# tum-vision/dvo_slam

Measured on NVIDIA H100. Metric: frame-pair alignments/sec @640x480x5-level, higher is better.
Workload: dtype f32

## Files before the change

dvo_slam_b200/csrc/stages.cuh:

```cuda
#pragma once
#include "common.cuh"
#include "f32x2.cuh"

namespace dvo_b200 {

constexpr unsigned kFullMask = 0xffffffffu;
constexpr int kConsumerWarps = kTileH;
constexpr int kCtaThreads = (kConsumerWarps + 1) * 32;
#ifndef DVO_WIN_COLS
#define DVO_WIN_COLS 152
#endif
#ifndef DVO_WIN_ROWS
#define DVO_WIN_ROWS 24
#endif
#ifndef DVO_STAGES
#define DVO_STAGES 2
#endif
constexpr int kWinCols = DVO_WIN_COLS;
constexpr int kWinRows = DVO_WIN_ROWS;
constexpr int kStages = DVO_STAGES;

__device__ __forceinline__ unsigned smem_u32(const void* p) { return (unsigned)__cvta_generic_to_shared(p); }
__device__ __forceinline__ void mbar_init(unsigned long long* bar, unsigned count) {
  asm volatile("mbarrier.init.shared::cta.b64 [%0], %1;" ::"r"(smem_u32(bar)), "r"(count) : "memory");
// ... 41 lines not shown
#if DVO_TRYWAIT_HINT_NS > 0
  asm volatile(
      "{\n\t.reg .pred p;\n\tmbarrier.try_wait.parity.acquire.cta.shared::cta.b64 p, [%1], %2, %3;\n\tselp.u32 %0, 1, 0, p;\n\t}"
      : "=r"(ok)
      : "r"(bar), "r"(parity), "r"((unsigned)DVO_TRYWAIT_HINT_NS)
      : "memory");
#else
  asm volatile(
      "{\n\t.reg .pred p;\n\tmbarrier.try_wait.parity.acquire.cta.shared::cta.b64 p, [%1], %2;\n\tselp.u32 %0, 1, 0, p;\n\t}"
      : "=r"(ok)
      : "r"(bar), "r"(parity)
      : "memory");
#endif
  return ok != 0;
}
__device__ __forceinline__ void mbar_wait_s(unsigned bar, unsigned parity, int* error_flag) {
  unsigned spins = 0;
  while (!mbar_try_wait_s(bar, parity)) {
    if (((++spins) & 0xfffu) == 0u) {
      if (*reinterpret_cast<volatile int*>(error_flag)) break;
      if (spins > (1u << 24)) { atomicExch(error_flag, 2); break; }
    }
  }
}
__device__ __forceinline__ void mbar_arrive_s(unsigned bar) {
  asm volatile("{\n\t.reg .b64 st;\n\tmbarrier.arrive.release.cta.shared::cta.b64 st, [%0];\n\t}" ::"r"(bar) : "memory");
}
__device__ __forceinline__ int4 lds_i4(unsigned addr) {
  int4 v;
  asm volatile("ld.shared.v4.b32 {%0, %1, %2, %3}, [%4];" : "=r"(v.x), "=r"(v.y), "=r"(v.z), "=r"(v.w) : "r"(addr));
  return v;
}

__device__ __forceinline__ void bulk_g2s(void* dst_smem, const void* src_gmem, unsigned bytes, unsigned long long* bar) {
  asm volatile("cp.async.bulk.shared::cta.global.mbarrier::complete_tx::bytes [%0], [%1], %2, [%3];" ::"r"(smem_u32(dst_smem)),
               "l"(src_gmem), "r"(bytes), "r"(smem_u32(bar))
               : "memory");
}
// ... 10 lines not shown
  return v;
}
__device__ __forceinline__ f2 lds_f2_at(unsigned addr) {
  f2 v;
  asm volatile("ld.shared.v2.f32 {%0, %1}, [%2];" : "=f"(v.x), "=f"(v.y) : "r"(addr));
  return v;
}

__device__ __forceinline__ unsigned pin(unsigned v) { asm volatile("" : "+r"(v)); return v; }
__device__ __forceinline__ int pin(int v) { asm volatile("" : "+r"(v)); return v; }
__device__ __forceinline__ float pin(float v) { asm volatile("" : "+f"(v)); return v; }
template <typename T>
__device__ __forceinline__ const T* pin(const T* p) { asm volatile("" : "+l"(p)); return p; }

struct __align__(16) TileDesc {
  int skip;
  int origin;
  int ulo, ucount;
  int vlo, vcount;
  int exact;
  int cmask;
};
struct __align__(128) StageBuf {
  float2 ref0[kTileH][kTileW];
  float tx[kTileW];
  float2 ref1[kTileH][kTileW];
  float2 win[kWinRows][kWinCols];
};
static_assert(offsetof(StageBuf, tx) == kRecTx * sizeof(float2) && offsetof(StageBuf, ref1) == kRecP1 * sizeof(float2) &&
              offsetof(StageBuf, win) == kRecF2 * sizeof(float2), "StageBuf must mirror the reference tile record");
struct TilePipe {
  StageBuf buf[kStages];
  unsigned long long full[kStages], empty[kStages];
  TileDesc desc[kStages];
};
static_assert(sizeof(TileDesc) == 32 && offsetof(TilePipe, desc) % 16 == 0, "TileDesc is read as two 16-byte words");

#ifdef DVO_PIPE_TIMING
struct PipeTiming {
  unsigned long long wait_full_a = 0, wait_full_b = 0, wait_empty = 0, produce = 0, rounds_a = 0, rounds_b = 0;
  unsigned long long tiles = 0, tiles_inexact = 0, tiles_skipped = 0, tiles_cmask = 0, slow_rounds = 0, rounds = 0;
  bool on = false;
};
#define DVO_CLOCK(tm) ((tm).on ? clock64() : 0)
#define DVO_ADD(tm, field, v) do { if ((tm).on) (tm).field += (v); } while (0)
#else
struct PipeTiming {};
#define DVO_CLOCK(tm) 0ll
#define DVO_ADD(tm, field, v) do { } while (0)
#endif

struct LevelGeom {
  int w, h, n, pitch;
  int nbands, nstrips;
  int strip0, strip_step, nmine;
};

struct StageConsts {
  f2 k0, k1, k2, k3;
  float k8, k9, k10, k11;
  f2 Pa, Pb;
  f2 cgh, cg, fxyh;
  float c_i, ubx, uby;
  int first_iteration;
};

__device__ __forceinline__ void load_stage_consts(const PairState& st, const PairLevel& pl, int w, int h, bool weights_from_prev,
                                                  StageConsts& c) {
  float kt[12], P[4];
#pragma unroll
  for (int i = 0; i < 12; ++i) kt[i] = __ldcg(&st.kt[i]);
#pragma unroll
  for (int i = 0; i < 4; ++i) P[i] = weights_from_prev ? __ldcg(&st.precision_prev[i]) : __ldcg(&st.precision[i]);
  c.k0 = pk(kt[0], kt[4]); c.k1 = pk(kt[1], kt[5]); c.k2 = pk(kt[2], kt[6]); c.k3 = pk(kt[3], kt[7]);
  c.k8 = kt[8]; c.k9 = kt[9]; c.k10 = kt[10]; c.k11 = kt[11];
  c.Pa = pk(P[0], P[1]); c.Pb = pk(P[2], P[3]);
  const float cgx = __fdiv_rn(__fmul_rn(0.5f, pl.cfx), 255.0f), cgy = __fdiv_rn(__fmul_rn(0.5f, pl.cfy), 255.0f);
  c.cg = pk(cgx, cgy);
  c.cgh = pk(0.5f * cgx, 0.5f * cgy);
  c.fxyh = pk(0.5f * pl.cfx, 0.5f * pl.cfy);
  c.c_i = 1.0f / 255.0f;
  c.ubx = pin((float)(w - 2)); c.uby = pin((float)(h - 2));
  c.first_iteration = __ldcg(&st.iteration) == 0;
}

template <bool kStageB, bool kCurMask = false>
__device__ __noinline__ void produce_tiles(TilePipe& tp, const PairLevel& pl, const LevelGeom& g, const StageConsts& c, unsigned tbase,
                                           int ntiles, int* error_flag, PipeTiming& tm) {
  const int lane = threadIdx.x & 31, sub = lane >> 3;
  const float2* cur = kStageB ? pl.c3 : pl.c0;
  int s_issue = g.strip0, b_issue = 0;
  for (int i0 = 0; i0 < ntiles; i0 += 4) {
    const long long tp0 = DVO_CLOCK(tm);
    unsigned wordA, wordD;
    {
      const int ii = min(i0 + sub, ntiles - 1);
      const int sd = ii / g.nbands;
      const int s = g.strip0 + sd * g.strip_step, b = ii - sd * g.nbands;
      const int y0 = s * kTileH, rows = min(kTileH, g.h - y0);
      const int x0 = b * kTileW, bw = min(kTileW, g.w - x0);
      const float2 zr = __ldg(pl.rrange + (size_t)s * g.nbands + b);
      const float txc = __ldg(pl.rtmpl + ((lane & 1) ? x0 + bw - 1 : x0));
      const float tyc = __ldg(pl.rtmpl + g.w + ((lane & 2) ? y0 + rows - 1 : y0));
      const bool has_depth = zr.x <= zr.y;
      const float z = (lane & 4) ? zr.y : zr.x;
      const float px = txc * z, py = tyc * z;
      const f2 XY = fma2(c.k0, bc(px), fma2(c.k1, bc(py), fma2(c.k2, bc(z), c.k3)));
      const float Zt = fmaf(c.k8, px, fmaf(c.k9, py, fmaf(c.k10, z, c.k11)));
      const float iz = 1.0f / Zt;
      float umin = lo(XY) * iz, vmin = hi(XY) * iz, umax = umin, vmax = vmin;
      const bool front_lane = Zt > 1e-6f && umin == umin && vmin == vmin;
#pragma unroll
      for (int off = 1; off < 8; off <<= 1) {
        umin = fminf(umin, __shfl_xor_sync(kFullMask, umin, off)); umax = fmaxf(umax, __shfl_xor_sync(kFullMask, umax, off));
        vmin = fminf(vmin, __shfl_xor_sync(kFullMask, vmin, off)); vmax = fmaxf(vmax, __shfl_xor_sync(kFullMask, vmax, off));
      }
      const bool front = ((__ballot_sync(kFullMask, front_lane) >> (sub * 8)) & 0xffu) == 0xffu;
      umin = fmaxf(umin, -8.f); vmin = fmaxf(vmin, -8.f); umax = fminf(umax, (float)g.w + 8.f); vmax = fminf(vmax, (float)g.h + 8.f);
// ... 24 lines not shown
        if (exact) {
          const int cx0 = bx0 >> 3, cx1 = (min(bx0 + ncols - 1, g.w - 1) >> 3) + 1;
          const int cy0 = max(row_lo, 0) >> 3, cy1 = (min(row_lo + nrows - 1, g.h - 1) >> 3) + 1;
          const int dirty = __ldg(csat + cy1 * sw + cx1) - __ldg(csat + cy0 * sw + cx1) - __ldg(csat + cy1 * sw + cx0) +
                            __ldg(csat + cy0 * sw + cx0);
          if (dirty) { exact = 0; cmask = 1; }
        } else {
          cmask = __ldg(csat + (sat_rows(g.h) - 1) * sw + sw - 1) != 0 ? 1 : 0;
        }
      }
      wordA = (unsigned)skip | ((unsigned)exact << 1) | ((unsigned)ncols << 2) | ((unsigned)nrows << 10) | ((unsigned)cmask << 31);
      wordD = (unsigned)bx0 | ((unsigned)(row_lo + 1) << 16);
    }
    DVO_ADD(tm, produce, DVO_CLOCK(tm) - tp0);
    const int kmax = min(4, ntiles - i0);
    for (int k = 0; k < kmax; ++k) {
      const unsigned t = tbase + (unsigned)(i0 + k);
      const int bufi = t % kStages;
      StageBuf& sb = tp.buf[bufi];
      const unsigned wa = __shfl_sync(kFullMask, wordA, k * 8), wd = __shfl_sync(kFullMask, wordD, k * 8);
      const int s = s_issue, b = b_issue;
      if (++b_issue == g.nbands) { b_issue = 0; s_issue += g.strip_step; }
      const int skip = (int)(wa & 1u), ncols = (int)((wa >> 2) & 0xffu), nrows = (int)((kCurMask ? wa & 0x7fffffffu : wa) >> 10);
      const int win_bx0 = (int)(wd & 0xffffu), win_row_lo = (int)(wd >> 16) - 1;
      TileDesc d;
      d.skip = skip; d.exact = (int)((wa >> 1) & 1u); d.cmask = kCurMask ? (int)(wa >> 31) : 0;
      d.origin = 0; d.ulo = 0; d.ucount = 0; d.vlo = 0; d.vcount = 0;
      if (ncols) {
        d.origin = (win_row_lo * kWinCols + win_bx0) * 8;
        d.ulo = win_bx0 == 0 ? 0 : win_bx0 + 1;
        const int uhi = (win_bx0 + ncols - 1 >= g.w - 1) ? g.w - 2 : win_bx0 + ncols - 3;
        d.ucount = max(uhi - d.ulo + 1, 0);
        d.vlo = win_row_lo + 1;
        d.vcount = max(nrows - 3, 0);
      }
      const unsigned win_row_bytes = (unsigned)ncols * 8u;
      const unsigned rec_bytes = (unsigned)(kStageB ? kRecF2 : kRecP1) * 8u;
      const unsigned total = skip ? 0u : rec_bytes + (unsigned)nrows * win_row_bytes;
      const long long tp1 = DVO_CLOCK(tm);
      mbar_wait(&tp.empty[bufi], ((t / kStages) & 1u) ^ 1u, error_flag);
      DVO_ADD(tm, wait_empty, DVO_CLOCK(tm) - tp1);
      DVO_ADD(tm, tiles, 1); DVO_ADD(tm, tiles_inexact, (!d.skip && !d.exact) ? 1 : 0); DVO_ADD(tm, tiles_skipped, d.skip ? 1 : 0);
      DVO_ADD(tm, tiles_cmask, d.cmask ? 1 : 0);
      if (lane == 0) {
        tp.desc[bufi] = d;
        if (total) mbar_arrive_expect_tx(&tp.full[bufi], total);
        else mbar_arrive(&tp.full[bufi]);
      }
      __syncwarp();
      if (!skip) {
        if (lane < nrows) {
          const int yy = min(max(win_row_lo + lane, 0), g.h - 1);
          bulk_g2s(&sb.win[lane][0], cur + (size_t)yy * g.pitch + win_bx0, win_row_bytes, &tp.full[bufi]);
        }
        if (lane == 31) bulk_g2s(&sb.ref0[0][0], pl.r0 + (size_t)(s * g.nbands + b) * kRecF2, rec_bytes, &tp.full[bufi]);
      }
    }
  }
}

struct PixelProjection {
  f2 f, gq;
  float Zt;
  int u0, v0;
  bool inb;
};

__device__ __forceinline__ PixelProjection project_pixel(float tx, float ty, float z, const StageConsts& c) {
  PixelProjection p;
  const f2 pxy = mul2(pk(tx, ty), bc(z));
  const float px = lo(pxy), py = hi(pxy);
  const f2 XY = fma2(c.k0, bc(px), fma2(c.k1, bc(py), fma2(c.k2, bc(z), c.k3)));
  p.Zt = __fmaf_rn(c.k8, px, __fmaf_rn(c.k9, py, __fmaf_rn(c.k10, z, c.k11)));
// ... 395 lines not shown
    }
    if (kCorrected && !kExact) {
      z0 = (r * 32 + lane == odd_col) ? odd_z : z0;
      z1 = (r * 32 + 32 + lane == odd_col) ? odd_z : z1;
    }
    const PixelProjection p0 = project_pixel(tx0, ty, z0, c);
    const PixelProjection p1 = project_pixel(tx1, ty, z1, c);
    float ei0, ez0, ei1, ez1;
    const bool v0 = residual_pixel<kExact>(p0, wv, ref_intensity<kAffine>(lo(rz0), br), z0, c, ei0, ez0);
    const bool v1 = residual_pixel<kExact>(p1, wv, ref_intensity<kAffine>(lo(rz1), br), z1, c, ei1, ez1);
    const float w0 = student_weight(c, first, ei0, ez0), w1 = student_weight(c, first, ei1, ez1);
    scale_add(ss, lane, lt_mask, v0, w0, ei0, ez0);
    scale_add(ss, lane, lt_mask, v1, w1, ei1, ez1);
  }
}
template <bool kCorrected, bool kAffine = false>
__device__ __forceinline__ void stage_a_run(TilePipe& tp, const PairLevel& pl, const LevelGeom& g, const StageConsts& c,
                                            float* row_exports, unsigned& tile_count, int* error_flag, PipeTiming& tm,
                                            const Brightness& br = {1.f, 0.f}) {
  const int lane = threadIdx.x & 31, q = threadIdx.x >> 5;
  const unsigned lt_mask = (1u << lane) - 1u;
  const int ntiles = g.nmine * g.nbands;
  const unsigned tbase = tile_count;
  tile_count += ntiles;
  if (q == kConsumerWarps) {
    produce_tiles<false>(tp, pl, g, c, tbase, ntiles, error_flag, tm);
    return;
  }
  int i = 0;
  const unsigned tp_s = pin(smem_u32(&tp));
  const unsigned my_ref = pin((unsigned)(offsetof(StageBuf, ref0) + (q * kTileW + lane) * 8));
  const unsigned my_tx = pin((unsigned)(offsetof(StageBuf, tx) + lane * 4));
  const int gw = pin(g.w), gh = pin(g.h), gnb = pin(g.nbands), gpitch = g.pitch;
  OddPoint odd;
  odd.y = -1; odd.x = 0; odd.z = 0.f;
  if (kCorrected) odd = load_odd_point(pl, g);
  for (int sk = 0, s = g.strip0; sk < g.nmine; ++sk, s += g.strip_step) {
    const int y = s * kTileH + q;
    const bool row_ok = y < gh;
    const float ty = __ldg(pl.rtmpl + gw + min(y, gh - 1));
    typename ScaleOf<kCorrected>::type ss;
    scale_state_init(ss);
    for (int b = 0; b < gnb; ++b, ++i) {
      const unsigned t = tbase + i;
      const unsigned bufi = t % kStages;
      const int x0 = b * kTileW, bw = min(kTileW, gw - x0);
      const long long tw0 = DVO_CLOCK(tm);
      mbar_wait_s(tp_s + (unsigned)offsetof(TilePipe, full) + bufi * 8u, (t / kStages) & 1u, error_flag);
      DVO_ADD(tm, wait_full_a, DVO_CLOCK(tm) - tw0);
      const unsigned bufs = tp_s + bufi * (unsigned)sizeof(StageBuf);
      const int4 d0 = lds_i4(tp_s + (unsigned)offsetof(TilePipe, desc) + bufi * 32u);
      if (row_ok && !d0.x) {
        const int4 d1 = lds_i4(tp_s + (unsigned)offsetof(TilePipe, desc) + bufi * 32u + 16u);
        const WinView wv = make_view(bufs, d0, d1, pl.c0, gw, gh, gpitch);
        const unsigned refa = bufs + my_ref, txa = bufs + my_tx;
        const bool odd_tile = kCorrected && y == odd.y && (unsigned)(odd.x - x0) < (unsigned)bw;
        if (wv.exact && bw == kTileW && !odd_tile) {
          if (c.first_iteration) stage_a_rounds<kCorrected, true, true, kAffine>(wv, bw, refa, txa, ty, c, ss, lane, lt_mask, -1, 0.f, br);
          else stage_a_rounds<kCorrected, true, false, kAffine>(wv, bw, refa, txa, ty, c, ss, lane, lt_mask, -1, 0.f, br);
        } else {
          stage_a_rounds<kCorrected, false, false, kAffine>(wv, bw, refa, txa, ty, c, ss, lane, lt_mask, odd_tile ? odd.x - x0 : -1,
                                                            odd.z, br);
        }
      }
      __syncwarp();
      if (lane == 0) mbar_arrive_s(tp_s + (unsigned)offsetof(TilePipe, empty) + bufi * 8u);
    }
    if (row_ok) scale_state_export(ss, lane, row_exports + (size_t)y * kSegExportFloats);
  }
}

struct StageBConsts {
  float P00, P01, P10, P11;
  float l, wd0, wd1;
};

template <int kCols> constexpr int kNormalValuesOf = 1 + kCols * (kCols + 1) / 2 + kCols;
constexpr int kNormalValues = kNormalValuesOf<6>;
constexpr int kNormalValuesAffine = kNormalValuesOf<8>;
template <bool kAffine> constexpr int kColsOf = kAffine ? 8 : 6;

template <int kCols>
__host__ __device__ constexpr int tri(int r, int c) { return r * kCols - r * (r - 1) / 2 + (c - r); }
template <int kCols>
// ... 145 lines not shown
      keep = valid && (rank + __popc(m & lt_mask)) < keep_rank;
      rank += __popc(m);
    }
    if (kDump && r * 32 < xlim) dump_record(dump, pix + r * 32, valid, E, G, H, z);
    const float ei = valid ? lo(E) : 0.f, ez = valid ? hi(E) : 0.f;
    const float wall = student_weight(c, first, ei, ez);
    const float wgt = valid ? wall : 0.f;
    stage_b_pixel(acc, cb, wgt, keep, ei, ez, valid ? G : bc(0.f), valid ? H : bc(0.f), valid ? z : 1.0f, valid ? tx : 0.f, ty,
                  valid ? lo(rz) : 0.f, -c.c_i);
  }
}

template <bool kDump, bool kCorrected, bool kCurMask = false, bool kAffine = false>
__device__ __forceinline__ void stage_b_run(TilePipe& tp, const PairLevel& pl, const LevelGeom& g, const StageConsts& c,
                                            const StageBConsts& cb, const int* row_base, const int* strip_base, long long n_keep,
                                            const RecordDump& dump, float* row_partial, unsigned& tile_count, int* error_flag,
                                            PipeTiming& tm, const Brightness& br = {1.f, 0.f}) {
  constexpr int kCols = kColsOf<kAffine>;
  const int lane = threadIdx.x & 31, q = threadIdx.x >> 5;
  const unsigned lt_mask = (1u << lane) - 1u;
  const int ntiles = g.nmine * g.nbands;
  const unsigned tbase = tile_count;
  tile_count += ntiles;
  if (q == kConsumerWarps) {
    produce_tiles<true, kCurMask>(tp, pl, g, c, tbase, ntiles, error_flag, tm);
    return;
  }
  int i = 0;
  const unsigned tp_s = pin(smem_u32(&tp));
  const unsigned my_ref = (unsigned)(offsetof(StageBuf, ref0) + (q * kTileW + lane) * 8);
  const unsigned my_tx = (unsigned)(offsetof(StageBuf, tx) + lane * 4);
  const int gw = g.w, gh = g.h, gnb = g.nbands, gpitch = g.pitch;
  OddPoint odd;
  odd.y = -1; odd.x = 0; odd.z = 0.f;
  if (kCorrected) odd = load_odd_point(pl, g);
  for (int sk = 0, s = g.strip0; sk < g.nmine; ++sk, s += g.strip_step) {
    const int y = s * kTileH + q;
    const bool row_ok = y < gh;
    const float ty = __ldg(pl.rtmpl + gw + min(y, gh - 1));
    bool cta_has_tail = false;
    int keep_rank = 0;
    int rank = 0;
    if (!kCorrected) {
      const long long sbase = __ldcg(strip_base + s);
      cta_has_tail = (long long)__ldcg(strip_base + s + 1) > n_keep;
      keep_rank = (int)max(min(n_keep - sbase, (long long)0x7fffffff), (long long)-1);
      if (cta_has_tail && row_ok) rank = __ldcg(row_base + y);
    }
    StageBAccN<kCols> acc;
    stage_b_init(acc);
    for (int b = 0; b < gnb; ++b, ++i) {
      const unsigned t = tbase + i;
      const unsigned bufi = t % kStages;
      const int x0 = b * kTileW, bw = min(kTileW, gw - x0);
      const long long tw0 = DVO_CLOCK(tm);
      mbar_wait_s(tp_s + (unsigned)offsetof(TilePipe, full) + bufi * 8u, (t / kStages) & 1u, error_flag);
      DVO_ADD(tm, wait_full_b, DVO_CLOCK(tm) - tw0);
      const unsigned bufs = tp_s + bufi * (unsigned)sizeof(StageBuf);
      const int4 d0 = lds_i4(tp_s + (unsigned)offsetof(TilePipe, desc) + bufi * 32u);
      if (row_ok && !d0.x) {
        const int4 d1 = lds_i4(tp_s + (unsigned)offsetof(TilePipe, desc) + bufi * 32u + 16u);
        const WinView wv = make_view(bufs, d0, d1, pl.c3, gw, gh, gpitch);
        const unsigned refa = bufs + my_ref, txa = bufs + my_tx;
        const size_t pix = (size_t)y * gw + x0 + lane;
        const bool odd_tile = kCorrected && y == odd.y && (unsigned)(odd.x - x0) < (unsigned)bw;
        if (wv.exact && bw == kTileW && !cta_has_tail && !odd_tile) {
          if (c.first_iteration)
            stage_b_rounds<kCorrected, true, true, kDump, false, kAffine>(wv, bw, refa, txa, ty, c, cb, acc, cta_has_tail, rank, keep_rank,
                                                                          dump, pix, lane, lt_mask, -1, 0.f, tm, false, nullptr, br);
          else
            stage_b_rounds<kCorrected, true, false, kDump, false, kAffine>(wv, bw, refa, txa, ty, c, cb, acc, cta_has_tail, rank, keep_rank,
                                                                           dump, pix, lane, lt_mask, -1, 0.f, tm, false, nullptr, br);
        } else {
          stage_b_rounds<kCorrected, false, false, kDump, kCurMask, kAffine>(wv, bw, refa, txa, ty, c, cb, acc, cta_has_tail, rank,
                                                                             keep_rank, dump, pix, lane, lt_mask,
                                                                             odd_tile ? odd.x - x0 : -1, odd.z, tm,
                                                                             kCurMask && d1.w != 0, pl.c0, br);
        }
      } else if (kDump && row_ok) {
        for (int xl = lane; xl < bw; xl += 32) dump_record(dump, (size_t)y * gw + x0 + xl, false, bc(0.f), bc(0.f), bc(0.f), 0.f);
      }
      __syncwarp();
      if (lane == 0) mbar_arrive_s(tp_s + (unsigned)offsetof(TilePipe, empty) + bufi * 8u);
    }
    if (row_ok) flush_row_partial(acc, lane, row_partial + (size_t)y * kNormalValuesOf<kCols>);
  }
}

__device__ __forceinline__ void load_stage_b_consts(const PairState& st, StageBConsts& c) {
  c.P00 = __ldcg(&st.precision[0]); c.P01 = __ldcg(&st.precision[1]); c.P10 = __ldcg(&st.precision[2]); c.P11 = __ldcg(&st.precision[3]);
  c.l = c.P01 / c.P00;
  c.wd0 = c.P00;
  c.wd1 = c.P11 - c.P01 * c.l;
}

}
```

dvo_slam_b200/csrc/tracker.cu:

```cuda
#include "common.cuh"
#include "stages.cuh"
#include "launch_plan.h"

#include <cstdio>
#include <cstring>
#include <limits>
#include <cmath>
#include <cstdlib>
#include <algorithm>
#include <type_traits>

namespace dvo_b200 {

namespace {

constexpr unsigned kFull = 0xffffffffu;
constexpr int kEndWarps = 4;

struct LevelLaunch {
  int w, h, n, pitch;
  int nbands, nstrips;
  int level_index;
  int level_id;
  int max_iterations;
// ... 349 lines not shown
    ls.has_inc = ls.num_iterations >= need;
  } else {
    st.inc = inc;
    st.initial_old = st.initial;
    st.initial = se3_mul(se3_inverse(inc), st.initial);
    st.estimate_old = st.estimate;
    st.estimate = estimate_new;
  }
  phase(5);
}

struct SquadState {
  int pair;
  unsigned arrive;
  unsigned phase;
  int pad_[29];
};

template <bool kAffine, bool kPrior = false>
struct LevelTailOf {
  using EndBase = typename std::conditional<kAffine, PairEndSmemAffine, PairEndSmem>::type;
  SegCombineSmem comb;
  typename std::conditional<kPrior, PairEndSmemPrior<EndBase>, EndBase>::type end;
  int s_flag[2];
};
template <bool kAffine, bool kPrior = false>
constexpr size_t kLevelSmemBytesOf = sizeof(TilePipe) + sizeof(LevelTailOf<kAffine, kPrior>);
constexpr size_t kLevelSmemBytes = kLevelSmemBytesOf<false>;

struct Segment {
  const PairLevel* pls;
  float* row_exports;
  int* row_base;
  double* strip_exports;
  int* strip_base;
  float* row_partial;
  double* strip_partial;
  SquadState* squads;
  int* queue;
  int* ready;
  int* ready_tail;
  int* arrivals;
  int cyclic;
  int pair_begin;
  int npairs_seg;
  unsigned long long* dbg2;
  unsigned long long* dbg;
  int nlev;
  int g, nsquads;
  int strips_per_cta[kMaxLevels];
  LevelLaunch lp[kMaxLevels];
};

struct PersistentArgs {
  PairState* states;
  int* error_flag;
  dvo_b200_iteration_stats* ilog;
  int max_log;
  const double* T_init;
  int skip_begin;
  float* dump;
  int npairs;
  int nseg;
  Segment seg[kMaxSeg];
  const PairLevel* pls0;
// ... 93 lines not shown
    cta_index = lt.s_flag[1];
    __syncthreads();
  }
  const int squad = cta_index / S.g, rank = cta_index - squad * S.g;
  if (squad >= S.nsquads) continue;
  SquadState* sq = S.squads + squad;
  int hmax = 0;
  for (int li = 0; li < S.nlev; ++li) hmax = max(hmax, S.lp[li].h);
  float* row_exports = S.row_exports + (size_t)squad * hmax * kSegExportFloats;
  int* row_base = S.row_base + (size_t)squad * hmax;
  const int smax = (hmax + kTileH - 1) / kTileH;
  double* strip_exports = S.strip_exports + (size_t)squad * smax * kStripExportDoubles;
  int* strip_base = S.strip_base + (size_t)squad * (smax + 1);
  float* row_partial = S.row_partial + (size_t)squad * hmax * kNV;
  double* strip_partial = S.strip_partial + (size_t)squad * smax * kNV;
  unsigned episode = 0;
  unsigned long long t_acc[8] = {0, 0, 0, 0, 0, 0, 0, 0}, t0 = 0, t1 = 0;
  const bool timing = S.dbg != nullptr && threadIdx.x == 0;
  PipeTiming tm;
#ifdef DVO_PIPE_TIMING
  tm.on = S.dbg != nullptr && lane == 0 && (warp == 0 || warp == kConsumerWarps);
#endif
  const unsigned long long t_start = timing ? global_ns() : 0;

  for (;;) {
    DVO_TICK();
    if (squad_arrive(sq, episode, S.g, lt.s_flag)) {
      if (threadIdx.x == 0) {
        int p = atomicAdd(S.queue, 1);
        if (p >= S.npairs_seg) p = -1;
// ... 20 lines not shown
    DVO_TOCK(6);
    const int pair = __ldcg(&sq->pair);
    if (pair < 0 || *reinterpret_cast<volatile int*>(a.error_flag)) break;
    PairState& st = a.states[pair];
    auto brightness = [&]() {
      Brightness br{1.f, 0.f};
      if constexpr (kAffine) br = Brightness{(float)__ldcg(&a.affine[pair].ab[0]), (float)__ldcg(&a.affine[pair].ab[1])};
      return br;
    };

    for (int li = 0; li < S.nlev; ++li) {
    const LevelLaunch& lp = S.lp[li];
    const typename LevelOf<kCurMask>::type pl = LevelOf<kCurMask>::load(a, S, (size_t)li * a.npairs + pair);
    LevelGeom geo;
    geo.w = lp.w; geo.h = lp.h; geo.n = lp.n; geo.pitch = lp.pitch; geo.nbands = lp.nbands; geo.nstrips = lp.nstrips;
    if (S.cyclic) {
      const int g_eff = min(S.g, lp.nstrips);
      geo.strip0 = min(rank, lp.nstrips); geo.strip_step = g_eff;
      geo.nmine = rank < g_eff ? (lp.nstrips - rank + g_eff - 1) / g_eff : 0;
    } else {
      geo.strip0 = min(rank * S.strips_per_cta[li], lp.nstrips); geo.strip_step = 1;
      geo.nmine = min(geo.strip0 + S.strips_per_cta[li], lp.nstrips) - geo.strip0;
    }
    if (!a.skip_begin) {
      if (squad_arrive(sq, episode, S.g, lt.s_flag)) {
        if (threadIdx.x == 0) {
          level_begin(st, pl, a.T_init, pair, lp);
          if constexpr (kAffine) {
            AffineState& af = a.affine[pair];
            af.ab_old[0] = af.ab[0]; af.ab_old[1] = af.ab[1];
          }
          squad_release(sq, episode);
        }
      } else {
        squad_wait(sq, episode, a.error_flag);
      }
      __syncthreads();
      ++episode;
      DVO_TOCK(6);
    }

    for (;;) {
      {
        StageConsts c;
        load_stage_consts(st, pl, lp.w, lp.h, false, c);
        const long long ts0 = DVO_CLOCK(tm);
        stage_a_run<kCorrected, kAffine>(tp, pl, geo, c, row_exports, tile_count, a.error_flag, tm, brightness());
        DVO_ADD(tm, rounds_a, DVO_CLOCK(tm) - ts0);
      }
      __syncthreads();
      for (int j = threadIdx.x; j < geo.nmine; j += kCtaThreads) {
        const int sj = geo.strip0 + j * geo.strip_step;
        combine_strip_rows(row_exports, sj * kTileH, min(sj * kTileH + kTileH, lp.h), row_base, strip_exports + (size_t)sj * kStripExportDoubles);
      }
      DVO_TOCK(0);
      if (squad_arrive(sq, episode, S.g, lt.s_flag)) {
        DVO_TOCK(2);
        if (warp == 0) {
          pair_mid_warp<kCorrected>(st, pair, strip_exports, strip_base, lp.nstrips, lp, a.ilog, a.max_log, lt.comb);
          if constexpr (kAffine) {
            AffineState& af = a.affine[pair];
            if (lane == 0 && !st.level_active) {
              af.ab[0] = af.ab_old[0]; af.ab[1] = af.ab_old[1];
              if (a.skip_begin) {
                for (int i = 0; i < 64; ++i) af.A[i] = 0.0;
                for (int i = 0; i < 8; ++i) af.b[i] = 0.0;
              }
            }
          }
          if (lane == 0) squad_release(sq, episode);
        }
        __syncthreads();
// ... 6 lines not shown
      ++episode;
      const bool failed = *reinterpret_cast<volatile int*>(a.error_flag) != 0;
      const bool level_ends = failed || !__ldcg(&st.level_active);
      if (level_ends && (!a.dump || failed)) break;

      {
        StageConsts c;
        load_stage_consts(st, pl, lp.w, lp.h, true, c);
        StageBConsts cb;
        load_stage_b_consts(st, cb);
        const long long n_keep = __ldcg(&st.n_keep);
        RecordDump dump;
        dump.planes = a.dump; dump.n = lp.n;
        const long long ts0 = DVO_CLOCK(tm);
        const Brightness br = brightness();
        if (a.dump) stage_b_run<true, kCorrected, kCurMask, kAffine>(tp, pl, geo, c, cb, row_base, strip_base, n_keep, dump, row_partial, tile_count, a.error_flag, tm, br);
        else stage_b_run<false, kCorrected, kCurMask, kAffine>(tp, pl, geo, c, cb, row_base, strip_base, n_keep, dump, row_partial, tile_count, a.error_flag, tm, br);
        DVO_ADD(tm, rounds_b, DVO_CLOCK(tm) - ts0);
      }
      __syncthreads();
      if (level_ends) break;
      for (int it = threadIdx.x; it < geo.nmine * kNV; it += kCtaThreads) {
        const int j = it / kNV, i = it - j * kNV;
        const int sj = geo.strip0 + j * geo.strip_step;
        const int nrow = min(kTileH, lp.h - sj * kTileH);
        const float* rp = row_partial + (size_t)sj * kTileH * kNV + i;
        float r[kTileH];
#pragma unroll
        for (int k = 0; k < kTileH; ++k) r[k] = k < nrow ? __ldcg(rp + (size_t)k * kNV) : 0.f;
        double v = 0.0;
#pragma unroll
        for (int k = 0; k < kTileH; ++k) v += (double)r[k];
        strip_partial[(size_t)sj * kNV + i] = v;
      }
      DVO_TOCK(1);
      if (squad_arrive(sq, episode, S.g, lt.s_flag)) {
        DVO_TOCK(3);
        if constexpr (kAffine) {
          if (threadIdx.x == 0) { lt.end.aff = a.affine + pair; lt.end.keep_system = a.skip_begin; }
// ... 95 lines not shown
  const double a = ab ? ab[2 * p] : 1.0, b = ab ? ab[2 * p + 1] : 0.0;
  s[p].ab[0] = a; s[p].ab[1] = b; s[p].ab_old[0] = a; s[p].ab_old[1] = b;
}

template <typename T>
int grow(dvo_b200_ctx* ctx, T*& ptr, size_t& cap, size_t need) {
  if (need <= cap) return 0;
  if (ptr) { cudaStreamSynchronize(ctx->stream); cudaFree(ptr); ptr = nullptr; cap = 0; }
  DVO_CUDA(ctx, cudaMalloc((void**)&ptr, need * sizeof(T)));
  cap = need;
  return 0;
}

struct ScratchLayout {
  size_t row_exports[kMaxSeg], row_base[kMaxSeg], strip_exports[kMaxSeg], strip_base[kMaxSeg], row_partial[kMaxSeg],
         strip_partial[kMaxSeg], squads[kMaxSeg];
  size_t counters;
  size_t ring;
  size_t bytes;
};

ScratchLayout scratch_layout(const PlanLaunch& L, int npairs, int nvals) {
  ScratchLayout o;
  size_t at = 0;
  auto take = [&](size_t bytes) { const size_t off = at; at += (bytes + 127) / 128 * 128; return off; };
  for (int s = 0; s < L.nseg; ++s) {
    const PlanSegment& S = L.seg[s];
    const size_t rows = (size_t)S.nsquads * S.hmax, strips = (size_t)S.nsquads * ((S.hmax + kTileH - 1) / kTileH);
    o.row_exports[s] = take(sizeof(float) * kSegExportFloats * rows);
    o.row_base[s] = take(sizeof(int) * rows);
    o.strip_exports[s] = take(sizeof(double) * kStripExportDoubles * strips);
    o.strip_base[s] = take(sizeof(int) * (strips + S.nsquads));
    o.row_partial[s] = take(sizeof(float) * nvals * rows);
    o.strip_partial[s] = take(sizeof(double) * nvals * strips);
  }
  for (int s = 0; s < L.nseg; ++s) o.squads[s] = take(sizeof(SquadState) * L.seg[s].nsquads);
  o.counters = take(sizeof(SquadState));
  o.ring = take(sizeof(int) * (size_t)npairs);
  o.bytes = at;
  return o;
}

int ensure_workspace(dvo_b200_ctx* ctx, int ndesc, const LaunchPlan& plan, int npairs, size_t dump_floats, int max_log_per_pair,
                     bool affine = false) {
  Workspace& ws = ctx->ws;
  if ((size_t)ndesc > ws.cap_pairs) {
    if (ws.d_pair_level) { cudaStreamSynchronize(ctx->stream); cudaFree(ws.d_pair_level); cudaFree(ws.d_state); }
    ws.d_pair_level = nullptr; ws.d_state = nullptr; ws.cap_pairs = 0;
    DVO_CUDA(ctx, cudaMalloc((void**)&ws.d_pair_level, sizeof(PairLevel) * ndesc + 16));
// ... 185 lines not shown
  pa.npairs = npairs; pa.nseg = L.nseg;
  pa.pls0 = ws.d_pair_level; pa.csat = ws.d_csat;
  pa.affine = affine ? ws.d_affine : nullptr;
  pa.prior = prior ? ws.d_prior : nullptr;
  for (int s = 0; s < L.nseg; ++s) {
    const PlanSegment& P = L.seg[s];
    Segment& S = pa.seg[s];
    S.pls = ws.d_pair_level + (size_t)P.first_li * npairs;
    S.row_exports = reinterpret_cast<float*>(base + o.row_exports[s]);
    S.row_base = reinterpret_cast<int*>(base + o.row_base[s]);
    S.strip_exports = reinterpret_cast<double*>(base + o.strip_exports[s]);
    S.strip_base = reinterpret_cast<int*>(base + o.strip_base[s]);
    S.row_partial = reinterpret_cast<float*>(base + o.row_partial[s]);
    S.strip_partial = reinterpret_cast<double*>(base + o.strip_partial[s]);
    S.squads = reinterpret_cast<SquadState*>(base + o.squads[s]);
    S.queue = counters + s; S.ready_tail = counters + kMaxSeg + s; S.arrivals = counters + 2 * kMaxSeg + s;
    S.ready = reinterpret_cast<int*>(base + o.ring) + P.pair_begin;
    S.cyclic = P.cyclic; S.pair_begin = P.pair_begin; S.npairs_seg = P.npairs;
    S.dbg = ctx->d_dbg ? ctx->d_dbg + 16 * (index + s) : nullptr;
    S.dbg2 = ctx->d_dbg ? ctx->d_dbg + 128 + 8 * (index + s) : nullptr;
    S.nlev = P.nlev; S.g = P.g; S.nsquads = P.nsquads;
    for (int k = 0; k < kMaxLevels; ++k) S.strips_per_cta[k] = P.strips_per_cta[k];
    for (int k = 0; k < P.nlev; ++k) {
      const int li = P.first_li + k;
      S.lp[k] = make_level_launch(levels[first - li], cfg, li, first - li);
    }
  }
  {
    ProfScope prof(ctx, 0);
    ProfScope prof_level(ctx, 8 + index);
    void* args[] = {&pa};
    const bool corrected = ctx->estimator == DVO_B200_ESTIMATOR_CORRECTED;
    DVO_CUDA(ctx, cudaLaunchCooperativeKernel(level_kernel(corrected, cur_mask, affine, prior), dim3(grid_ctas(ctx, affine, prior)),
                                              dim3(kCtaThreads), args, level_smem_bytes(affine, prior), st));
    ctx->launches++;
  }
  DVO_CUDA(ctx, cudaMemcpyAsync(&ws.h_active[index], pa.error_flag, sizeof(int), cudaMemcpyDeviceToHost, st));
// ... 219 lines not shown
```

Measured before the change: 21260.

## Replace static strip partitioning with dynamic atomic strip claiming per squad

Replaces the fixed cyclic or blocked assignment of image strips to CTAs with dynamic claiming: each producer warp grabs further strips from a per-squad atomic counter and records them in a claim list. Consumers learn strip identity and tail status from the tile descriptor, and a sentinel descriptor ends the stage. The per-row ty values and the strip tail check now come from the producer through shared memory instead of per-warp global loads. The aim is to balance load across CTAs when strip cost varies, at the cost of atomics, an extra end-of-stage pipeline slot, and claim-counter resets.

```diff
diff --git a/dvo_slam_b200/csrc/stages.cuh b/dvo_slam_b200/csrc/stages.cuh
--- a/dvo_slam_b200/csrc/stages.cuh
+++ b/dvo_slam_b200/csrc/stages.cuh
@@ -79,14 +79,15 @@
 #endif
   return ok != 0;
 }
-__device__ __forceinline__ void mbar_wait_s(unsigned bar, unsigned parity, int* error_flag) {
+__device__ __forceinline__ bool mbar_wait_s(unsigned bar, unsigned parity, int* error_flag) {
   unsigned spins = 0;
   while (!mbar_try_wait_s(bar, parity)) {
     if (((++spins) & 0xfffu) == 0u) {
-      if (*reinterpret_cast<volatile int*>(error_flag)) break;
-      if (spins > (1u << 24)) { atomicExch(error_flag, 2); break; }
-    }
-  }
+      if (*reinterpret_cast<volatile int*>(error_flag)) return false;
+      if (spins > (1u << 24)) { atomicExch(error_flag, 2); return false; }
+    }
+  }
+  return true;
 }
 __device__ __forceinline__ void mbar_arrive_s(unsigned bar) {
   asm volatile("{\n\t.reg .b64 st;\n\tmbarrier.arrive.release.cta.shared::cta.b64 st, [%0];\n\t}" ::"r"(bar) : "memory");
@@ -127,7 +128,7 @@
 __device__ __forceinline__ const T* pin(const T* p) { asm volatile("" : "+l"(p)); return p; }
 
 struct __align__(16) TileDesc {
-  int skip;
+  int strip_skip;
   int origin;
   int ulo, ucount;
   int vlo, vcount;
@@ -146,8 +147,11 @@
   StageBuf buf[kStages];
   unsigned long long full[kStages], empty[kStages];
   TileDesc desc[kStages];
-};
+  float ty[kStages][kTileH];
+};
+static_assert(kTileH <= 8, "produce_tiles loads a strip's ty values in groups of eight lanes");
 static_assert(sizeof(TileDesc) == 32 && offsetof(TilePipe, desc) % 16 == 0, "TileDesc is read as two 16-byte words");
+constexpr int kStageEnd = -1;
 
 #ifdef DVO_PIPE_TIMING
 struct PipeTiming {
@@ -166,8 +170,15 @@
 struct LevelGeom {
   int w, h, n, pitch;
   int nbands, nstrips;
-  int strip0, strip_step, nmine;
-};
+};
+
+struct StripClaims {
+  int g, rank;
+  int* next;
+  int* list;
+  int* count;
+};
+__device__ __forceinline__ int claimed_strip(const StripClaims& cl, int j) { return j == 0 ? cl.rank : cl.list[j]; }
 
 struct StageConsts {
   f2 k0, k1, k2, k3;
@@ -198,23 +209,49 @@
 }
 
 template <bool kStageB, bool kCurMask = false>
-__device__ __noinline__ void produce_tiles(TilePipe& tp, const PairLevel& pl, const LevelGeom& g, const StageConsts& c, unsigned tbase,
-                                           int ntiles, int* error_flag, PipeTiming& tm) {
+__device__ __noinline__ unsigned produce_tiles(TilePipe& tp, const PairLevel& pl, const LevelGeom& g, const StageConsts& c,
+                                               unsigned tbase, const StripClaims& cl, const int* strip_base, long long n_keep,
+                                               int* error_flag, PipeTiming& tm) {
   const int lane = threadIdx.x & 31, sub = lane >> 3;
   const float2* cur = kStageB ? pl.c3 : pl.c0;
-  int s_issue = g.strip0, b_issue = 0;
-  for (int i0 = 0; i0 < ntiles; i0 += 4) {
+  int nclaimed = 0;
+  int held = 0;
+  bool drained = false;
+  auto take = [&](int s) {
+    if (s >= g.nstrips) { drained = true; return; }
+    if (lane == (nclaimed & 31)) held = s;
+    if (lane == 0 && nclaimed > 0) cl.list[nclaimed] = s;
+    ++nclaimed;
+  };
+  int next_local = cl.rank + cl.g;
+  auto claim = [&]() {
+    int s = 0;
+    if (cl.g == 1) s = next_local++;
+    else if (lane == 0) s = cl.g + atomicAdd(cl.next, 1);
+    take(__shfl_sync(kFullMask, s, 0));
+  };
+  take(cl.rank);
+  if (cl.g >= g.nstrips) drained = true;
+  int sd_issue = 0, b_issue = 0;
+  for (int i0 = 0;;) {
     const long long tp0 = DVO_CLOCK(tm);
+    while (!drained && nclaimed * g.nbands < i0 + (cl.g == 1 ? 4 : 1)) claim();
+    const int ntiles = nclaimed * g.nbands;
+    if (i0 >= ntiles) break;
     unsigned wordA, wordD;
+    float ty_row;
+    int tail = 0;
     {
       const int ii = min(i0 + sub, ntiles - 1);
       const int sd = ii / g.nbands;
-      const int s = g.strip0 + sd * g.strip_step, b = ii - sd * g.nbands;
+      const int s = __shfl_sync(kFullMask, held, sd & 31), b = ii - sd * g.nbands;
       const int y0 = s * kTileH, rows = min(kTileH, g.h - y0);
       const int x0 = b * kTileW, bw = min(kTileW, g.w - x0);
       const float2 zr = __ldg(pl.rrange + (size_t)s * g.nbands + b);
       const float txc = __ldg(pl.rtmpl + ((lane & 1) ? x0 + bw - 1 : x0));
       const float tyc = __ldg(pl.rtmpl + g.w + ((lane & 2) ? y0 + rows - 1 : y0));
+      ty_row = __ldg(pl.rtmpl + g.w + min(y0 + (lane & 7), g.h - 1));
+      if (kStageB && strip_base) tail = (long long)__ldcg(strip_base + s + 1) > n_keep;
       const bool has_depth = zr.x <= zr.y;
       const float z = (lane & 4) ? zr.y : zr.x;
       const float px = txc * z, py = tyc * z;
@@ -269,17 +306,22 @@
     }
     DVO_ADD(tm, produce, DVO_CLOCK(tm) - tp0);
     const int kmax = min(4, ntiles - i0);
+    int ahead = 0;
+    const bool claim_ahead = cl.g > 1 && !drained && ntiles < i0 + kmax + 4;
+    if (claim_ahead && lane == 0) ahead = cl.g + atomicAdd(cl.next, 1);
     for (int k = 0; k < kmax; ++k) {
       const unsigned t = tbase + (unsigned)(i0 + k);
       const int bufi = t % kStages;
       StageBuf& sb = tp.buf[bufi];
       const unsigned wa = __shfl_sync(kFullMask, wordA, k * 8), wd = __shfl_sync(kFullMask, wordD, k * 8);
-      const int s = s_issue, b = b_issue;
-      if (++b_issue == g.nbands) { b_issue = 0; s_issue += g.strip_step; }
+      const float tyv = __shfl_sync(kFullMask, ty_row, k * 8 + (lane & 7));
+      const int tail_k = __shfl_sync(kFullMask, tail, k * 8);
+      const int s = __shfl_sync(kFullMask, held, sd_issue & 31), b = b_issue;
+      if (++b_issue == g.nbands) { b_issue = 0; ++sd_issue; }
       const int skip = (int)(wa & 1u), ncols = (int)((wa >> 2) & 0xffu), nrows = (int)((kCurMask ? wa & 0x7fffffffu : wa) >> 10);
       const int win_bx0 = (int)(wd & 0xffffu), win_row_lo = (int)(wd >> 16) - 1;
       TileDesc d;
-      d.skip = skip; d.exact = (int)((wa >> 1) & 1u); d.cmask = kCurMask ? (int)(wa >> 31) : 0;
+      d.strip_skip = skip | (tail_k << 1) | (s << 2); d.exact = (int)((wa >> 1) & 1u); d.cmask = kCurMask ? (int)(wa >> 31) : 0;
       d.origin = 0; d.ulo = 0; d.ucount = 0; d.vlo = 0; d.vcount = 0;
       if (ncols) {
         d.origin = (win_row_lo * kWinCols + win_bx0) * 8;
@@ -295,8 +337,10 @@
       const long long tp1 = DVO_CLOCK(tm);
       mbar_wait(&tp.empty[bufi], ((t / kStages) & 1u) ^ 1u, error_flag);
       DVO_ADD(tm, wait_empty, DVO_CLOCK(tm) - tp1);
-      DVO_ADD(tm, tiles, 1); DVO_ADD(tm, tiles_inexact, (!d.skip && !d.exact) ? 1 : 0); DVO_ADD(tm, tiles_skipped, d.skip ? 1 : 0);
+      DVO_ADD(tm, tiles, 1); DVO_ADD(tm, tiles_inexact, (!skip && !d.exact) ? 1 : 0); DVO_ADD(tm, tiles_skipped, skip ? 1 : 0);
       DVO_ADD(tm, tiles_cmask, d.cmask ? 1 : 0);
+      if (lane < kTileH) tp.ty[bufi][lane] = tyv;
+      __syncwarp();
       if (lane == 0) {
         tp.desc[bufi] = d;
         if (total) mbar_arrive_expect_tx(&tp.full[bufi], total);
@@ -311,7 +355,19 @@
         if (lane == 31) bulk_g2s(&sb.ref0[0][0], pl.r0 + (size_t)(s * g.nbands + b) * kRecF2, rec_bytes, &tp.full[bufi]);
       }
     }
-  }
+    if (claim_ahead) take(__shfl_sync(kFullMask, ahead, 0));
+    i0 += kmax;
+  }
+  const unsigned ntiles = (unsigned)(nclaimed * g.nbands);
+  const unsigned t = tbase + ntiles;
+  const int bufi = t % kStages;
+  mbar_wait(&tp.empty[bufi], ((t / kStages) & 1u) ^ 1u, error_flag);
+  if (lane == 0) {
+    tp.desc[bufi].strip_skip = kStageEnd;
+    *cl.count = nclaimed;
+    mbar_arrive(&tp.full[bufi]);
+  }
+  return ntiles + 1u;
 }
 
 struct PixelProjection {
@@ -737,20 +793,28 @@
     scale_add(ss, lane, lt_mask, v1, w1, ei1, ez1);
   }
 }
+__device__ __forceinline__ int next_strip_head(unsigned tp_s, unsigned t, int* error_flag) {
+  const unsigned bufi = t % kStages;
+  if (!mbar_wait_s(tp_s + (unsigned)offsetof(TilePipe, full) + bufi * 8u, (t / kStages) & 1u, error_flag)) return kStageEnd;
+  return lds_i4(tp_s + (unsigned)offsetof(TilePipe, desc) + bufi * 32u).x;
+}
+__device__ __forceinline__ void end_stage_slot(unsigned tp_s, unsigned t) {
+  __syncwarp();
+  if ((threadIdx.x & 31) == 0) mbar_arrive_s(tp_s + (unsigned)offsetof(TilePipe, empty) + (t % kStages) * 8u);
+}
+
 template <bool kCorrected, bool kAffine = false>
 __device__ __forceinline__ void stage_a_run(TilePipe& tp, const PairLevel& pl, const LevelGeom& g, const StageConsts& c,
-                                            float* row_exports, unsigned& tile_count, int* error_flag, PipeTiming& tm,
-                                            const Brightness& br = {1.f, 0.f}) {
+                                            float* row_exports, const StripClaims& cl, unsigned& tile_count, int* error_flag,
+                                            PipeTiming& tm, const Brightness& br = {1.f, 0.f}) {
   const int lane = threadIdx.x & 31, q = threadIdx.x >> 5;
   const unsigned lt_mask = (1u << lane) - 1u;
-  const int ntiles = g.nmine * g.nbands;
   const unsigned tbase = tile_count;
-  tile_count += ntiles;
   if (q == kConsumerWarps) {
-    produce_tiles<false>(tp, pl, g, c, tbase, ntiles, error_flag, tm);
+    tile_count += produce_tiles<false>(tp, pl, g, c, tbase, cl, nullptr, 0, error_flag, tm);
     return;
   }
-  int i = 0;
+  unsigned i = 0;
   const unsigned tp_s = pin(smem_u32(&tp));
   const unsigned my_ref = pin((unsigned)(offsetof(StageBuf, ref0) + (q * kTileW + lane) * 8));
   const unsigned my_tx = pin((unsigned)(offsetof(StageBuf, tx) + lane * 4));
@@ -758,10 +822,14 @@
   OddPoint odd;
   odd.y = -1; odd.x = 0; odd.z = 0.f;
   if (kCorrected) odd = load_odd_point(pl, g);
-  for (int sk = 0, s = g.strip0; sk < g.nmine; ++sk, s += g.strip_step) {
-    const int y = s * kTileH + q;
+  for (;;) {
+    const long long th0 = DVO_CLOCK(tm);
+    const int head = next_strip_head(tp_s, tbase + i, error_flag);
+    DVO_ADD(tm, wait_full_a, DVO_CLOCK(tm) - th0);
+    if (head < 0) { end_stage_slot(tp_s, tbase + i); ++i; break; }
+    const int y = (head >> 2) * kTileH + q;
     const bool row_ok = y < gh;
-    const float ty = __ldg(pl.rtmpl + gw + min(y, gh - 1));
+    const float ty = lds_f32(tp_s + (unsigned)offsetof(TilePipe, ty) + (((tbase + i) % kStages) * kTileH + q) * 4u);
     typename ScaleOf<kCorrected>::type ss;
     scale_state_init(ss);
     for (int b = 0; b < gnb; ++b, ++i) {
@@ -773,7 +841,7 @@
       DVO_ADD(tm, wait_full_a, DVO_CLOCK(tm) - tw0);
       const unsigned bufs = tp_s + bufi * (unsigned)sizeof(StageBuf);
       const int4 d0 = lds_i4(tp_s + (unsigned)offsetof(TilePipe, desc) + bufi * 32u);
-      if (row_ok && !d0.x) {
+      if (row_ok && !(d0.x & 1)) {
         const int4 d1 = lds_i4(tp_s + (unsigned)offsetof(TilePipe, desc) + bufi * 32u + 16u);
         const WinView wv = make_view(bufs, d0, d1, pl.c0, gw, gh, gpitch);
         const unsigned refa = bufs + my_ref, txa = bufs + my_tx;
@@ -791,6 +859,7 @@
     }
     if (row_ok) scale_state_export(ss, lane, row_exports + (size_t)y * kSegExportFloats);
   }
+  tile_count += i;
 }
 
 struct StageBConsts {
@@ -966,19 +1035,17 @@
 template <bool kDump, bool kCorrected, bool kCurMask = false, bool kAffine = false>
 __device__ __forceinline__ void stage_b_run(TilePipe& tp, const PairLevel& pl, const LevelGeom& g, const StageConsts& c,
                                             const StageBConsts& cb, const int* row_base, const int* strip_base, long long n_keep,
-                                            const RecordDump& dump, float* row_partial, unsigned& tile_count, int* error_flag,
-                                            PipeTiming& tm, const Brightness& br = {1.f, 0.f}) {
+                                            const RecordDump& dump, float* row_partial, const StripClaims& cl,
+                                            unsigned& tile_count, int* error_flag, PipeTiming& tm, const Brightness& br = {1.f, 0.f}) {
   constexpr int kCols = kColsOf<kAffine>;
   const int lane = threadIdx.x & 31, q = threadIdx.x >> 5;
   const unsigned lt_mask = (1u << lane) - 1u;
-  const int ntiles = g.nmine * g.nbands;
   const unsigned tbase = tile_count;
-  tile_count += ntiles;
   if (q == kConsumerWarps) {
-    produce_tiles<true, kCurMask>(tp, pl, g, c, tbase, ntiles, error_flag, tm);
+    tile_count += produce_tiles<true, kCurMask>(tp, pl, g, c, tbase, cl, kCorrected ? nullptr : strip_base, n_keep, error_flag, tm);
     return;
   }
-  int i = 0;
+  unsigned i = 0;
   const unsigned tp_s = pin(smem_u32(&tp));
   const unsigned my_ref = (unsigned)(offsetof(StageBuf, ref0) + (q * kTileW + lane) * 8);
   const unsigned my_tx = (unsigned)(offsetof(StageBuf, tx) + lane * 4);
@@ -986,18 +1053,23 @@
   OddPoint odd;
   odd.y = -1; odd.x = 0; odd.z = 0.f;
   if (kCorrected) odd = load_odd_point(pl, g);
-  for (int sk = 0, s = g.strip0; sk < g.nmine; ++sk, s += g.strip_step) {
+  for (;;) {
+    const long long th0 = DVO_CLOCK(tm);
+    const int head = next_strip_head(tp_s, tbase + i, error_flag);
+    DVO_ADD(tm, wait_full_b, DVO_CLOCK(tm) - th0);
+    if (head < 0) { end_stage_slot(tp_s, tbase + i); ++i; break; }
+    const int s = head >> 2;
     const int y = s * kTileH + q;
     const bool row_ok = y < gh;
-    const float ty = __ldg(pl.rtmpl + gw + min(y, gh - 1));
+    const float ty = lds_f32(tp_s + (unsigned)offsetof(TilePipe, ty) + (((tbase + i) % kStages) * kTileH + q) * 4u);
     bool cta_has_tail = false;
     int keep_rank = 0;
     int rank = 0;
-    if (!kCorrected) {
+    if (!kCorrected && ((head >> 1) & 1)) {
+      cta_has_tail = true;
       const long long sbase = __ldcg(strip_base + s);
-      cta_has_tail = (long long)__ldcg(strip_base + s + 1) > n_keep;
       keep_rank = (int)max(min(n_keep - sbase, (long long)0x7fffffff), (long long)-1);
-      if (cta_has_tail && row_ok) rank = __ldcg(row_base + y);
+      if (row_ok) rank = __ldcg(row_base + y);
     }
     StageBAccN<kCols> acc;
     stage_b_init(acc);
@@ -1010,7 +1082,7 @@
       DVO_ADD(tm, wait_full_b, DVO_CLOCK(tm) - tw0);
       const unsigned bufs = tp_s + bufi * (unsigned)sizeof(StageBuf);
       const int4 d0 = lds_i4(tp_s + (unsigned)offsetof(TilePipe, desc) + bufi * 32u);
-      if (row_ok && !d0.x) {
+      if (row_ok && !(d0.x & 1)) {
         const int4 d1 = lds_i4(tp_s + (unsigned)offsetof(TilePipe, desc) + bufi * 32u + 16u);
         const WinView wv = make_view(bufs, d0, d1, pl.c3, gw, gh, gpitch);
         const unsigned refa = bufs + my_ref, txa = bufs + my_tx;
@@ -1037,6 +1109,7 @@
     }
     if (row_ok) flush_row_partial(acc, lane, row_partial + (size_t)y * kNormalValuesOf<kCols>);
   }
+  tile_count += i;
 }
 
 __device__ __forceinline__ void load_stage_b_consts(const PairState& st, StageBConsts& c) {
diff --git a/dvo_slam_b200/csrc/tracker.cu b/dvo_slam_b200/csrc/tracker.cu
--- a/dvo_slam_b200/csrc/tracker.cu
+++ b/dvo_slam_b200/csrc/tracker.cu
@@ -387,7 +387,8 @@
   int pair;
   unsigned arrive;
   unsigned phase;
-  int pad_[29];
+  int claim[2];
+  int pad_[27];
 };
 
 template <bool kAffine, bool kPrior = false>
@@ -396,6 +397,7 @@
   SegCombineSmem comb;
   typename std::conditional<kPrior, PairEndSmemPrior<EndBase>, EndBase>::type end;
   int s_flag[2];
+  int n_claimed;
 };
 template <bool kAffine, bool kPrior = false>
 constexpr size_t kLevelSmemBytesOf = sizeof(TilePipe) + sizeof(LevelTailOf<kAffine, kPrior>);
@@ -410,18 +412,17 @@
   float* row_partial;
   double* strip_partial;
   SquadState* squads;
+  int* claims;
   int* queue;
   int* ready;
   int* ready_tail;
   int* arrivals;
-  int cyclic;
   int pair_begin;
   int npairs_seg;
   unsigned long long* dbg2;
   unsigned long long* dbg;
   int nlev;
   int g, nsquads;
-  int strips_per_cta[kMaxLevels];
   LevelLaunch lp[kMaxLevels];
 };
 
@@ -545,6 +546,8 @@
   int* strip_base = S.strip_base + (size_t)squad * (smax + 1);
   float* row_partial = S.row_partial + (size_t)squad * hmax * kNV;
   double* strip_partial = S.strip_partial + (size_t)squad * smax * kNV;
+  int* const claimed = S.claims + (size_t)cta_index * smax;
+  const StripClaims claims_a{S.g, rank, &sq->claim[0], claimed, &lt.n_claimed}, claims_b{S.g, rank, &sq->claim[1], claimed, &lt.n_claimed};
   unsigned episode = 0;
   unsigned long long t_acc[8] = {0, 0, 0, 0, 0, 0, 0, 0}, t0 = 0, t1 = 0;
   const bool timing = S.dbg != nullptr && threadIdx.x == 0;
@@ -595,14 +598,6 @@
     const typename LevelOf<kCurMask>::type pl = LevelOf<kCurMask>::load(a, S, (size_t)li * a.npairs + pair);
     LevelGeom geo;
     geo.w = lp.w; geo.h = lp.h; geo.n = lp.n; geo.pitch = lp.pitch; geo.nbands = lp.nbands; geo.nstrips = lp.nstrips;
-    if (S.cyclic) {
-      const int g_eff = min(S.g, lp.nstrips);
-      geo.strip0 = min(rank, lp.nstrips); geo.strip_step = g_eff;
-      geo.nmine = rank < g_eff ? (lp.nstrips - rank + g_eff - 1) / g_eff : 0;
-    } else {
-      geo.strip0 = min(rank * S.strips_per_cta[li], lp.nstrips); geo.strip_step = 1;
-      geo.nmine = min(geo.strip0 + S.strips_per_cta[li], lp.nstrips) - geo.strip0;
-    }
     if (!a.skip_begin) {
       if (squad_arrive(sq, episode, S.g, lt.s_flag)) {
         if (threadIdx.x == 0) {
@@ -626,17 +621,18 @@
         StageConsts c;
         load_stage_consts(st, pl, lp.w, lp.h, false, c);
         const long long ts0 = DVO_CLOCK(tm);
-        stage_a_run<kCorrected, kAffine>(tp, pl, geo, c, row_exports, tile_count, a.error_flag, tm, brightness());
+        stage_a_run<kCorrected, kAffine>(tp, pl, geo, c, row_exports, claims_a, tile_count, a.error_flag, tm, brightness());
         DVO_ADD(tm, rounds_a, DVO_CLOCK(tm) - ts0);
       }
       __syncthreads();
-      for (int j = threadIdx.x; j < geo.nmine; j += kCtaThreads) {
-        const int sj = geo.strip0 + j * geo.strip_step;
+      for (int j = threadIdx.x; j < lt.n_claimed; j += kCtaThreads) {
+        const int sj = claimed_strip(claims_a, j);
         combine_strip_rows(row_exports, sj * kTileH, min(sj * kTileH + kTileH, lp.h), row_base, strip_exports + (size_t)sj * kStripExportDoubles);
       }
       DVO_TOCK(0);
       if (squad_arrive(sq, episode, S.g, lt.s_flag)) {
         DVO_TOCK(2);
+        if (threadIdx.x == 0) { sq->claim[0] = 0; sq->claim[1] = 0; }
         if (warp == 0) {
           pair_mid_warp<kCorrected>(st, pair, strip_exports, strip_base, lp.nstrips, lp, a.ilog, a.max_log, lt.comb);
           if constexpr (kAffine) {
@@ -673,15 +669,15 @@
         dump.planes = a.dump; dump.n = lp.n;
         const long long ts0 = DVO_CLOCK(tm);
         const Brightness br = brightness();
-        if (a.dump) stage_b_run<true, kCorrected, kCurMask, kAffine>(tp, pl, geo, c, cb, row_base, strip_base, n_keep, dump, row_partial, tile_count, a.error_flag, tm, br);
-        else stage_b_run<false, kCorrected, kCurMask, kAffine>(tp, pl, geo, c, cb, row_base, strip_base, n_keep, dump, row_partial, tile_count, a.error_flag, tm, br);
+        if (a.dump) stage_b_run<true, kCorrected, kCurMask, kAffine>(tp, pl, geo, c, cb, row_base, strip_base, n_keep, dump, row_partial, claims_b, tile_count, a.error_flag, tm, br);
+        else stage_b_run<false, kCorrected, kCurMask, kAffine>(tp, pl, geo, c, cb, row_base, strip_base, n_keep, dump, row_partial, claims_b, tile_count, a.error_flag, tm, br);
         DVO_ADD(tm, rounds_b, DVO_CLOCK(tm) - ts0);
       }
       __syncthreads();
       if (level_ends) break;
-      for (int it = threadIdx.x; it < geo.nmine * kNV; it += kCtaThreads) {
+      for (int it = threadIdx.x; it < lt.n_claimed * kNV; it += kCtaThreads) {
         const int j = it / kNV, i = it - j * kNV;
-        const int sj = geo.strip0 + j * geo.strip_step;
+        const int sj = claimed_strip(claims_b, j);
         const int nrow = min(kTileH, lp.h - sj * kTileH);
         const float* rp = row_partial + (size_t)sj * kTileH * kNV + i;
         float r[kTileH];
@@ -807,7 +803,7 @@
 
 struct ScratchLayout {
   size_t row_exports[kMaxSeg], row_base[kMaxSeg], strip_exports[kMaxSeg], strip_base[kMaxSeg], row_partial[kMaxSeg],
-         strip_partial[kMaxSeg], squads[kMaxSeg];
+         strip_partial[kMaxSeg], claims[kMaxSeg], squads[kMaxSeg];
   size_t counters;
   size_t ring;
   size_t bytes;
@@ -826,6 +822,7 @@
     o.strip_base[s] = take(sizeof(int) * (strips + S.nsquads));
     o.row_partial[s] = take(sizeof(float) * nvals * rows);
     o.strip_partial[s] = take(sizeof(double) * nvals * strips);
+    o.claims[s] = take(sizeof(int) * S.g * strips);
   }
   for (int s = 0; s < L.nseg; ++s) o.squads[s] = take(sizeof(SquadState) * L.seg[s].nsquads);
   o.counters = take(sizeof(SquadState));
@@ -1041,13 +1038,13 @@
     S.row_partial = reinterpret_cast<float*>(base + o.row_partial[s]);
     S.strip_partial = reinterpret_cast<double*>(base + o.strip_partial[s]);
     S.squads = reinterpret_cast<SquadState*>(base + o.squads[s]);
+    S.claims = reinterpret_cast<int*>(base + o.claims[s]);
     S.queue = counters + s; S.ready_tail = counters + kMaxSeg + s; S.arrivals = counters + 2 * kMaxSeg + s;
     S.ready = reinterpret_cast<int*>(base + o.ring) + P.pair_begin;
-    S.cyclic = P.cyclic; S.pair_begin = P.pair_begin; S.npairs_seg = P.npairs;
+    S.pair_begin = P.pair_begin; S.npairs_seg = P.npairs;
     S.dbg = ctx->d_dbg ? ctx->d_dbg + 16 * (index + s) : nullptr;
     S.dbg2 = ctx->d_dbg ? ctx->d_dbg + 128 + 8 * (index + s) : nullptr;
     S.nlev = P.nlev; S.g = P.g; S.nsquads = P.nsquads;
-    for (int k = 0; k < kMaxLevels; ++k) S.strips_per_cta[k] = P.strips_per_cta[k];
     for (int k = 0; k < P.nlev; ++k) {
       const int li = P.first_li + k;
       S.lp[k] = make_level_launch(levels[first - li], cfg, li, first - li);
```

Result: faster. 21640 (median of 6 runs) (+1.8%).
